# mishapadidar/GP-Derivatives-Variational-Inference

Measured on NVIDIA B200. Metric: DSVGP train points/s (ELBO fwd+bwd), higher is better.
Workload: dtype f32

## Files before the change

gp-derivatives-variational-inference_b200/csrc/api.cu:

```cuda
#include "../../include/dsvgp_b200.h"
#include "chol.cuh"
#include "common.cuh"
#include "data.cuh"
#include "gemm.cuh"
#include "kdir.cuh"
#include "misc.cuh"
#include "optim.cuh"
#include "tc_prep.cuh"
#include "trmm_tc.cuh"

using namespace dsvgp;
#define ST(s) reinterpret_cast<cudaStream_t>(s)

namespace dsvgp { unsigned long long g_launch_count = 0; }
namespace dsvgp { extern int g_fwd_tib, g_fwd_stream_stores, g_bwd_vpl; }

extern "C" {

int dsvgp_version(void) { return 100; }
int64_t dsvgp_launch_count(void) { return (int64_t)dsvgp::g_launch_count; }
int dsvgp_set_kdir_bwd_vpl(int vpl) {
  if (vpl == 2 || vpl == 4) dsvgp::g_bwd_vpl = vpl;
  return dsvgp::g_bwd_vpl;
}
int dsvgp_set_kdir_fwd_knobs(int tib, int stream_stores) {
  const int old = dsvgp::g_fwd_tib * 4 + dsvgp::g_fwd_stream_stores;
  if (tib == 0 || (tib >= 8 && tib <= 64 && tib % 8 == 0)) dsvgp::g_fwd_tib = tib;
  if (stream_stores >= 0 && stream_stores <= 2) dsvgp::g_fwd_stream_stores = stream_stores;
  return old;
}
int dsvgp_built_for_sm(void) { return 100; }

int dsvgp_hyp_from_raw_f32(const float* a, const float* b, const float* c, const float* d, double* hyp, dsvgp_stream_t s) { return hyp_from_raw<float>(a, b, c, d, hyp, ST(s)); }
int dsvgp_hyp_from_raw_f64(const double* a, const double* b, const double* c, const double* d, double* hyp, dsvgp_stream_t s) { return hyp_from_raw<double>(a, b, c, d, hyp, ST(s)); }

int dsvgp_normalize_dirs_f32(const float* v, int rows, int d, float* vh, float* inv, dsvgp_stream_t s) { return normalize_dirs<float, float>(v, rows, d, vh, inv, ST(s)); }
int dsvgp_normalize_dirs_f64(const double* v, int rows, int d, double* vh, double* inv, dsvgp_stream_t s) { return normalize_dirs<double, double>(v, rows, d, vh, inv, ST(s)); }
int dsvgp_normalize_dirs_f32f64(const float* v, int rows, int d, double* vh, double* inv, dsvgp_stream_t s) { return normalize_dirs<float, double>(v, rows, d, vh, inv, ST(s)); }

int dsvgp_normalize_dirs_canon_f32(const float* v, int rows, int d, float* vh, float* inv, int* cidx, int* canon_flag, dsvgp_stream_t s) {
  if (!cidx || !canon_flag) return DSVGP_ERR_ARG;
  return normalize_dirs<float, float>(v, rows, d, vh, inv, ST(s), cidx, canon_flag);
}
int dsvgp_kdir_fwd_canon_f32(const float* x1, const float* u1, int n1, int p1, const float* x2, const float* w2, const int* cidx2, const int* canon_flag, int n2, int p2, int d, const double* hyp, int use_os, double diag_add, float* K, int64_t ldk, float* Klo, dsvgp_stream_t s) {
  if (!x1 || !x2 || !hyp || !K || (p1 > 0 && !u1) || (p2 > 0 && !w2)) return DSVGP_ERR_ARG;
  return kdir_fwd<float, float>(x1, u1, n1, p1, x2, w2, n2, p2, d, hyp, use_os, diag_add, K, ldk, ST(s), cidx2, canon_flag, Klo);
}

#define KFWD(NAME, T, TK)                                                                                          \
  int NAME(const T* x1, const TK* u1, int n1, int p1, const T* x2, const TK* w2, int n2, int p2, int d,            \
           const double* hyp, int use_os, double diag_add, TK* K, int64_t ldk, dsvgp_stream_t s) {                 \
    if (!x1 || !x2 || !hyp || !K || (p1 > 0 && !u1) || (p2 > 0 && !w2)) return DSVGP_ERR_ARG;                     \
    return kdir_fwd<T, TK>(x1, u1, n1, p1, x2, w2, n2, p2, d, hyp, use_os, diag_add, K, ldk, ST(s));               \
  }
KFWD(dsvgp_kdir_fwd_f32, float, float)
KFWD(dsvgp_kdir_fwd_f64, double, double)
KFWD(dsvgp_kdir_fwd_f32f64, float, double)

int dsvgp_kdir_diag_f32(int n, int p, const double* hyp, int use_os, float* out, dsvgp_stream_t s) { return kdir_diag<float>(n, p, hyp, use_os, out, ST(s)); }
int dsvgp_kdir_diag_f64(int n, int p, const double* hyp, int use_os, double* out, dsvgp_stream_t s) { return kdir_diag<double>(n, p, hyp, use_os, out, ST(s)); }

size_t dsvgp_kdir_bwd_workspace_f32(int n1, int p1, int n2, int p2, int d) { return kdir_bwd_workspace<float>(n1, p1, n2, p2, d); }
size_t dsvgp_kdir_bwd_workspace_f64(int n1, int p1, int n2, int p2, int d) { return kdir_bwd_workspace<double>(n1, p1, n2, p2, d); }

#define KBWD(NAME, T, TK)                                                                                          \
  int NAME(const T* x1, const TK* u1, const TK* inv1, int n1, int p1, const T* x2, const TK* w2, int n2, int p2,   \
           int d, const double* hyp, int use_os, const TK* dK, int64_t lddk, int dk_trans, double scale,           \
           double* gx, double* gv, double* gsc, void* ws, size_t ws_bytes, dsvgp_stream_t s) {                     \
                                                \
    if (!x1 || !x2 || !hyp || !dK || !ws || (p1 > 0 && (!u1 || (gv && !inv1))) || (p2 > 0 && !w2)) return DSVGP_ERR_ARG; \
    return kdir_bwd<T, TK>(x1, u1, inv1, n1, p1, x2, w2, n2, p2, d, hyp, use_os, dK, lddk, dk_trans, scale, gx,    \
                           gv, gsc, ws, ws_bytes, ST(s));                                                          \
  }
KBWD(dsvgp_kdir_bwd_f32, float, float)
KBWD(dsvgp_kdir_bwd_f64, double, double)
KBWD(dsvgp_kdir_bwd_f32f64, float, double)

void dsvgp_chol_plan(int Mq, int* Mp, int* nb0, int* nlev) { chol_plan(Mq, Mp, nb0, nlev); }
int dsvgp_pad_identity_f64(double* A, int64_t ld, int Mq, int Mp, dsvgp_stream_t s) { return pad_identity(A, ld, Mq, Mp, ST(s)); }
int dsvgp_chol_f64(double* Awork, int64_t lda, double* L, int64_t ldl, double* W, int64_t ldw, int Mp, int nb0, int nlev, int* info, dsvgp_stream_t s) {
  return chol_factor_inverse(Awork, lda, L, ldl, W, ldw, Mp, nb0, nlev, info, ST(s));
}

int dsvgp_set_potrf_debug(void* p) { set_potrf_debug(static_cast<long long*>(p)); return 0; }
int dsvgp_collect_grads_f32(const double* small, int nZ, int nV, const double* hyp, int noise_mode, float* out, dsvgp_stream_t s) { return collect_grads<float>(small, nZ, nV, hyp, noise_mode, out, ST(s)); }
int dsvgp_collect_grads_f64(const double* small, int nZ, int nV, const double* hyp, int noise_mode, double* out, dsvgp_stream_t s) { return collect_grads<double>(small, nZ, nV, hyp, noise_mode, out, ST(s)); }
int dsvgp_set_gemm64_async(int on) { set_gemm64_async(on); return get_gemm64_async(); }
int dsvgp_set_rank_update(int on) { set_rank_update(on); return get_rank_update(); }
int dsvgp_set_chol_variant(int v) { set_chol_variant(v); return get_chol_variant(); }
int dsvgp_set_chol_lookahead(int on) { set_chol_lookahead(on); return get_chol_lookahead(); }
int dsvgp_set_chol_mid_link(int k) { set_chol_mid_link(k); return get_chol_mid_link(); }
int dsvgp_chol_wait_mid(dsvgp_stream_t s) { return chol_wait_mid(reinterpret_cast<cudaStream_t>(s)); }
int dsvgp_set_chol_inv_streams(int n) { set_chol_inv_streams(n); return get_chol_inv_streams(); }
int dsvgp_set_chol_graph(int on) { set_chol_graph(on); return get_chol_graph(); }
int dsvgp_set_chol_priority(int on) { set_chol_priority(on); return get_chol_priority(); }

int dsvgp_gemm_f32(int ta, int tb, int M, int N, int K, double alpha, const float* A, int64_t lda, const float* B, int64_t ldb, double beta, float* C, int64_t ldc, int a_tri, int b_tri, int c_tri, int batch, int64_t sA, int64_t sB, int64_t sC, const float* D, int64_t ldd, float* C2, int64_t ldc2, const float* D2, int64_t ldd2, dsvgp_stream_t s) {
  return gemm<float>(ta != 0, tb != 0, M, N, K, (float)alpha, A, lda, B, ldb, (float)beta, C, ldc, a_tri, b_tri, c_tri, batch, sA, sB, sC, ST(s), D, ldd, C2, ldc2, D2, ldd2);
}
int dsvgp_gemm_f64(int ta, int tb, int M, int N, int K, double alpha, const double* A, int64_t lda, const double* B, int64_t ldb, double beta, double* C, int64_t ldc, int a_tri, int b_tri, int c_tri, int batch, int64_t sA, int64_t sB, int64_t sC, const double* D, int64_t ldd, double* C2, int64_t ldc2, const double* D2, int64_t ldd2, dsvgp_stream_t s) {
  return gemm<double>(ta != 0, tb != 0, M, N, K, alpha, A, lda, B, ldb, beta, C, ldc, a_tri, b_tri, c_tri, batch, sA, sB, sC, ST(s), D, ldd, C2, ldc2, D2, ldd2);
}

int dsvgp_absmax_f32(const float* x, int64_t ld, int rows, int cols, int mode, unsigned int* out_bits, dsvgp_stream_t s) { return absmax<float>(x, ld, rows, cols, mode, out_bits, ST(s)); }
int dsvgp_absmax_f64(const double* x, int64_t ld, int rows, int cols, int mode, unsigned int* out_bits, dsvgp_stream_t s) { return absmax<double>(x, ld, rows, cols, mode, out_bits, ST(s)); }
int dsvgp_tc_scales_f32(const double* hyp, double jitter, const unsigned int* maxbits, int Mq, float* scales, int stage, dsvgp_stream_t s) { return tc_scales(hyp, jitter, maxbits, Mq, scales, stage, ST(s)); }
int dsvgp_split_half_f32(const float* src, int64_t lds, int rows, int cols, int mode, const float* scale, void* hi, void* lo, int64_t ldh, void* hiT, void* loT, int64_t ldhT, dsvgp_stream_t s) { return split_half<float>(src, lds, rows, cols, mode, scale, hi, lo, ldh, hiT, loT, ldhT, ST(s)); }
int dsvgp_split_half_f64(const double* src, int64_t lds, int rows, int cols, int mode, const float* scale, void* hi, void* lo, int64_t ldh, void* hiT, void* loT, int64_t ldhT, dsvgp_stream_t s) { return split_half<double>(src, lds, rows, cols, mode, scale, hi, lo, ldh, hiT, loT, ldhT, ST(s)); }
int dsvgp_build_d_split_f32(const float* E, int64_t lde, const float* P, int64_t ldp, int n, const float* scale, void* hi, void* lo, int64_t ldh, dsvgp_stream_t s) { return build_d_split(E, lde, P, ldp, n, scale, hi, lo, ldh, ST(s)); }
int dsvgp_build_d_absmax_f32(const float* E, int64_t lde, const float* P, int64_t ldp, int n, unsigned int* out_bits, dsvgp_stream_t s) { return build_d_absmax(E, lde, P, ldp, n, out_bits, ST(s)); }
int dsvgp_kdir_fwd_half_f32(const float* x1, const float* u1, int n1, int p1, const float* x2, const float* w2, const int* cidx2, const int* canon_flag, int n2, int p2, int d, const double* hyp, int use_os, double diag_add, float* K, int64_t ldk, void* Kh, void* Kl, int64_t ldkh, const float* hscale, dsvgp_stream_t s) {
  if (!x1 || !x2 || !hyp || !K || !Kh || !Kl || !hscale || (p1 > 0 && !u1) || (p2 > 0 && !w2)) return DSVGP_ERR_ARG;
  return kdir_fwd<float, float>(x1, u1, n1, p1, x2, w2, n2, p2, d, hyp, use_os, diag_add, K, ldk, ST(s), cidx2, canon_flag, nullptr, Kh, Kl, ldkh, hscale);
}
int dsvgp_dA_half_f32(const float* A, const float* C, int64_t ld, int rows, int nq, const float* m, const float* gmu, const float* gvar, float* tp, int nslab, float* t, void* dAh, void* dAl, void* Agh, void* Agl, int64_t ldh, const float* s_dA, const float* s_Ag, dsvgp_stream_t s) {
  if (!A || !C || !m || !gmu || !gvar || !tp || !t || !dAh || !dAl || !Agh || !Agl || !s_dA || !s_Ag) return DSVGP_ERR_ARG;
  return dA_apply_half(A, C, ld, rows, nq, m, gmu, gvar, tp, nslab, t, dAh, dAl, Agh, Agl, ldh, s_dA, s_Ag, nullptr, nullptr, nullptr, ST(s));
}
int dsvgp_dA_half_h_f32(const void* Ah, const void* Al, const float* a_scale, const float* C, int64_t ld, int rows, int nq, const float* m, const float* gmu, const float* gvar, float* tp, int nslab, float* t, void* dAh, void* dAl, void* Agh, void* Agl, int64_t ldh, const float* s_dA, const float* s_Ag, dsvgp_stream_t s) {
  if (!Ah || !Al || !a_scale || !C || !m || !gmu || !gvar || !tp || !t || !dAh || !dAl || !Agh || !Agl || !s_dA || !s_Ag) return DSVGP_ERR_ARG;
  return dA_apply_half(nullptr, C, ld, rows, nq, m, gmu, gvar, tp, nslab, t, dAh, dAl, Agh, Agl, ldh, s_dA, s_Ag, Ah, Al, a_scale, ST(s));
}
int dsvgp_col_dots_h_f32(const void* Ah, const void* Al, int64_t ldh, const float* a_scale, const float* C, int64_t ld, int rows, int nq, const float* m, float* pm, float* pv, int nslab, unsigned int* cmax_bits, dsvgp_stream_t s) {
  if (!m || !pm || !pv) return DSVGP_ERR_ARG;
  return col_dots_half(Ah, Al, ldh, a_scale, C, ld, rows, nq, m, pm, pv, nslab, cmax_bits, ST(s));
}
int dsvgp_gemm_tch_supported_f32(const void* A, int64_t lda, const void* B, int64_t ldb, int b_kmajor, int N) { return gemm_tch_supported(A, lda, B, ldb, b_kmajor, N); }
int dsvgp_gemm_tch_f32(const void* Ah, const void* Al, int64_t lda, const void* Bh, const void* Bl, int64_t ldb, int b_kmajor, int M, int N, int K, double alpha, double beta, const float* ab_inv, float* C, int64_t ldc, const float* D, int64_t ldd, float* C2, int64_t ldc2, const float* D2, int64_t ldd2, void* Ch, void* Cl, int64_t ldch, const float* c_scale, void* C2h, void* C2l, int64_t ldc2h, const float* c2_scale, int a_tri, int c_lower, int chunk, int nsplit, float* split_ws, dsvgp_stream_t s) {
  return gemm_tch(Ah, Al, lda, Bh, Bl, ldb, b_kmajor, M, N, K, (float)alpha, (float)beta, ab_inv, C, ldc, D, ldd, C2, ldc2, D2, ldd2, Ch, Cl, ldch, c_scale, C2h, C2l, ldc2h, c2_scale, a_tri, c_lower, chunk, nsplit, split_ws, ST(s));
}
int dsvgp_gemm_tc_supported_f32(const float* A, int64_t lda, const float* B, int64_t ldb, int b_kmajor, int N) { return gemm_tc_supported(A, lda, B, ldb, b_kmajor, N); }
int dsvgp_gemm_tc_f32(const float* Ah, const float* Al, int64_t lda, const float* Bh, const float* Bl, int64_t ldb, int b_kmajor, int M, int N, int K, double alpha, double beta, float* C, int64_t ldc, const float* D, int64_t ldd, float* C2, int64_t ldc2, const float* D2, int64_t ldd2, int a_tri, int c_lower, int chunk, float* Clo, float* C2lo, int nsplit, float* split_ws, dsvgp_stream_t s) {
  return gemm_tc(Ah, Al, lda, Bh, Bl, ldb, b_kmajor, M, N, K, (float)alpha, (float)beta, C, ldc, D, ldd, C2, ldc2, D2, ldd2, a_tri, c_lower, chunk, Clo, C2lo, nsplit, split_ws, ST(s));
}
int dsvgp_set_tc_tile_n(int n) { set_tc_tile_n(n); return get_tc_tile_n(); }
int dsvgp_set_tc_max_pairs(int n) { set_tc_max_pairs(n); return get_tc_max_pairs(); }
int dsvgp_set_tc_persistent(int on) { set_tc_persistent(on); return get_tc_persistent(); }
int dsvgp_set_tc_trace(void* buf, int cap_items) { set_tc_trace(static_cast<long long*>(buf), cap_items); return DSVGP_OK; }
int dsvgp_tc_work_list(int M, int N, int K, int a_tri, int c_lower, int nsplit, int pairs, int bke, int* out, int cap) {
  if (M <= 0 || N <= 0 || K <= 0 || nsplit < 1 || pairs < 1 || bke < 1 || cap < 0 || (cap > 0 && !out)) return DSVGP_ERR_ARG;
  const std::vector<int> t = tc::build_sched(M, N, K, a_tri, c_lower, nsplit, pairs, bke, nullptr);
  for (int i = 0; i < cap && i < (int)t.size(); ++i) out[i] = t[i];
  return (int)t.size();
}
int dsvgp_set_tc_cta_group(int cg) { set_tc_cta_group(cg); return get_tc_cta_group(); }
int dsvgp_split_lo_f32(const float* x, int64_t ldx, float* lo, int64_t ldl, int rows, int cols, dsvgp_stream_t s) { return split_lo(x, ldx, lo, ldl, rows, cols, ST(s)); }
int dsvgp_transpose_f32(const float* src, int64_t lds, float* dst, int64_t ldd, int rows, int cols, dsvgp_stream_t s) { return transpose_f32(src, lds, dst, ldd, rows, cols, ST(s)); }

// ... 73 lines not shown
```

gp-derivatives-variational-inference_b200/csrc/build.py:

```python
import os
import subprocess
import sys
from concurrent.futures import ThreadPoolExecutor

HERE = os.path.dirname(os.path.abspath(__file__))
OUT = os.path.join(os.path.dirname(HERE), "dsvgp_b200", "libdsvgp_b200.so")
SOURCES = ["kdir.cu", "gemm.cu", "chol.cu", "misc.cu", "optim.cu", "data.cu", "tc_prep.cu", "trmm_tc.cu", "api.cu"]
NVCC = os.environ.get("NVCC", "/usr/local/cuda/bin/nvcc")
FLAGS = ["-gencode", "arch=compute_100a,code=sm_100a", "-lineinfo", "-O3", "-std=c++17",
         "-Xcompiler", "-fPIC", "--expt-relaxed-constexpr"]


def _newer(a, b):
    return not os.path.exists(b) or os.path.getmtime(a) > os.path.getmtime(b)


def build(force=False, verbose=False):
    bdir = os.path.join(HERE, "build")
    os.makedirs(bdir, exist_ok=True)
    headers = [os.path.join(HERE, f) for f in os.listdir(HERE) if f.endswith((".cuh", ".h"))]
    headers.append(os.path.join(os.path.dirname(os.path.dirname(HERE)), "include", "dsvgp_b200.h"))
    srcs = [s for s in SOURCES if os.path.exists(os.path.join(HERE, s))]
    objs, jobs = [], []
    for s in srcs:
        src, obj = os.path.join(HERE, s), os.path.join(bdir, s[:-3] + ".o")
        objs.append(obj)
        if force or _newer(src, obj) or any(_newer(h, obj) for h in headers):
            jobs.append([NVCC, *FLAGS, *(["-Xptxas", "-v"] if verbose else []), "-c", src, "-o", obj])

    def run(cmd):
        r = subprocess.run(cmd, capture_output=True, text=True)
        if r.returncode != 0:
            raise RuntimeError("nvcc failed: " + " ".join(cmd) + "\n" + r.stdout + r.stderr)
        if verbose:
            sys.stderr.write(r.stderr)

    with ThreadPoolExecutor(max_workers=min(6, max(1, len(jobs)))) as ex:
        list(ex.map(run, jobs))
    if jobs or not os.path.exists(OUT):
        run([NVCC, "-shared", "-gencode", "arch=compute_100a,code=sm_100a", "-o", OUT, *objs])
    return OUT


if __name__ == "__main__":
    print(build(force="--force" in sys.argv, verbose="-v" in sys.argv))
```

gp-derivatives-variational-inference_b200/dsvgp_b200/_lib.py:

```python
import ctypes
import os
import re

import torch

_HERE = os.path.dirname(os.path.abspath(__file__))
LIB_PATH = os.path.join(_HERE, "libdsvgp_b200.so")
HEADER_PATH = os.path.normpath(os.path.join(_HERE, "..", "..", "include", "dsvgp_b200.h"))

_CTYPES = {"int": ctypes.c_int, "int64_t": ctypes.c_int64, "double": ctypes.c_double, "size_t": ctypes.c_size_t,
           "dsvgp_stream_t": ctypes.c_void_p, "void": None}
_PROTO = re.compile(r"^(int|void|size_t|int64_t)\s+(dsvgp_\w+)\s*\(([^;]*)\)\s*;", re.M)

ERRORS = {-1: "DSVGP_ERR_ARG (bad argument)", -2: "DSVGP_ERR_LAUNCH (CUDA launch failed)",
          -3: "DSVGP_ERR_WORKSPACE (workspace too small)"}


class DsvgpError(RuntimeError):
    pass


def parse_header(path=HEADER_PATH):
    protos = {}
    with open(path) as f:
        text = f.read()
    for ret, name, args in _PROTO.findall(text):
        argtypes = []
        args = args.strip()
        if args and args != "void":
            for a in args.split(","):
                a = a.strip()
                if "*" in a:
                    argtypes.append(ctypes.c_void_p)
                else:
                    argtypes.append(_CTYPES[a.replace("const ", "").split()[0]])
        protos[name] = (_CTYPES[ret], argtypes)
    return protos


PROTOTYPES = parse_header()

if not os.path.exists(LIB_PATH):
    raise ImportError(
        f"{LIB_PATH} is missing: build it with `python gp-derivatives-variational-inference_b200/csrc/build.py` "
        "(or __graft_entry__.build()).  dsvgp_b200 has no CPU or PyTorch fallback.")
_lib = ctypes.CDLL(LIB_PATH)
for _name, (_ret, _args) in PROTOTYPES.items():
    _fn = getattr(_lib, _name)
    _fn.restype = _ret
    _fn.argtypes = _args


def _arg(a):
    if a is None:
        return None
    if isinstance(a, torch.Tensor):
        if not a.is_cuda:
            raise DsvgpError("dsvgp_b200 kernels take CUDA tensors only (there is no CPU path)")
        return ctypes.c_void_p(a.data_ptr())
    return a


_RAW_STREAM = getattr(torch._C, "_cuda_getCurrentRawStream", None)
_GET_DEVICE = getattr(torch._C, "_cuda_getDevice", None)

# ... 56 lines not shown
```

gp-derivatives-variational-inference_b200/dsvgp_b200/engine.py:

```python
import os

import torch

from . import ops
from .ops import F32, F64, TRI_LOWER, TRI_UPPER

KZZ_JITTER = 1e-3
PRED_JITTER = 1e-4
CHOL_RETRY = (1e-6, 1e-5, 1e-4)
USE_TC = True
USE_FP16 = True
DENSE_D = True
WHITEN_FP64 = "auto"
WHITEN_FP64_MAX_NQ = 2048
DEFER_SIDE_WORK = True
TC_CHUNK = 2
TCH_CHUNK = 1
WORKSPACE_CACHE = 6
PERSISTENT_UNDER_REDUCE = os.environ.get("DSVGP_PERSISTENT_UNDER_REDUCE", "1") != "0"
HALF_A = False
F16 = torch.float16
_PARAM_NAMES = ("Z", "Vz", "m", "Ls_raw", "c", "raw_os", "raw_ell", "raw_noise")


# ... 70 lines not shown
        if self.tc:
            if not self.tch:
                self.lo1, self.lo2, self.lo3 = (e(Mq, self.ldn) for _ in range(3))
            self.E_lo, self.ET, self.ET_lo = sq(), sq(), sq()
            sg = lambda: e(Mq, self.ldg)[:, :Mq]
            self.G_lo, self.H_lo = sg(), sg()
            self.syrk_split = max(1, min(8, self.nq // 4096))
            self.split_ws = e(self.syrk_split * Mq * _round_up(Mq, 4)) if self.syrk_split > 1 else None
        self.nslab = max(1, ops.reduce_slabs(Mq, nq))
        self.pm, self.pv = e(self.nslab, nq), e(self.nslab, nq)
        self.mu, self.var, self.gmu, self.gvar = e(nq), e(nq), e(nq), e(nq)
        self.tp = e(max(1, min(64, nq // 2048)), Mq)
        self.big = torch.zeros(Mq * self.ldg + Mq, dtype=T, device=device)
        self.G, self.t = self.big[: Mq * self.ldg].view(Mq, self.ldg)[:, :Mq], self.big[Mq * self.ldg:]
        self.small = torch.zeros(8 + M * d + M * p * d, dtype=F64, device=device)
        self.sc = self.small[:8]
        self.gZ = self.small[8: 8 + M * d].view(M, d)
        self.gVz = self.small[8 + M * d:].view(M * p, d) if p else None
        self.small2 = torch.zeros_like(self.small)
        self.gZ2 = self.small2[8: 8 + M * d].view(M, d)
        self.gVz2 = self.small2[8 + M * d:].view(M * p, d) if p else None
        self.kl = torch.zeros(1, dtype=F64, device=device)
        self.scratch = e(max(8192, 2 * ((nq + 255) // 256) + 64), dt=F64)
        self.scratch_kl = e(512, dt=F64)
        self.H = e(Mq, self.ldg)[:, :Mq] if T == F32 else sq()
        self.X = sq()
        self.Y, self.Psi, self.S = (e(Mq, Mq, dt=F64) for _ in range(3))
        self.gm = self.gLs = None
        self.wx = None
        self.generation = 0
        self.canon = None


class Engine:
    def __init__(self):
        self._ws, self._fac, self._streams, self._events = {}, {}, {}, {}

    def _fork_event(self, device):
        key = str(device)
        ev = self._events.get(key)
        if ev is None:
            ev = self._events[key] = torch.cuda.Event()
        return ev

    def _scales_event(self, device):
        key = "scales:" + str(device)
        ev = self._events.get(key)
        if ev is None:
            ev = self._events[key] = torch.cuda.Event()
        return ev

    def _side_stream(self, device):
        key = str(device)
        st = self._streams.get(key)
        if st is None:
            st = self._streams[key] = torch.cuda.Stream(device=device)
        return st

    def workspace(self, device, dtype, n, d, M, p, p2):
        key = (str(device), dtype, n, d, M, p, p2)
        ws = self._ws.pop(key, None)
        if ws is None:
            while len(self._ws) >= WORKSPACE_CACHE:
                self._ws.pop(next(iter(self._ws)))
            ws = Workspace(device, dtype, n, d, M, p, p2)
        self._ws[key] = ws
        ws.generation += 1
        return ws

    def factor(self, device, dtype, d, M, p):
        key = (str(device), dtype, d, M, p)
        f = self._fac.pop(key, None)
        if f is None:
            while len(self._fac) >= WORKSPACE_CACHE:
                self._fac.pop(next(iter(self._fac)))
            f = Factor(device, dtype, d, M, p)
        self._fac[key] = f
        f.generation += 1
        return f

    @staticmethod
    def _validate(P, x, Vx, p, p2, y=None):
        if x.dim() != 2:
            raise ValueError(f"x must be (n, d); got {tuple(x.shape)}")
        if not x.is_cuda:
            raise TypeError("dsvgp_b200 runs on CUDA tensors only (there is no CPU path)")
        T, dev = x.dtype, x.device
        if T not in (F32, F64):
            raise TypeError(f"unsupported dtype {T}: the hot path is built for float32 and float64")
        n, d = x.shape
        M = P.Z.shape[0]
        Mq = M * (p + 1)
        want = {"Z": (M, d), "Vz": (M * p, d) if p else None, "m": (Mq,), "Ls_raw": (Mq, Mq)}
        for name in _PARAM_NAMES:
            t = getattr(P, name, None)
            if t is None:
                continue
            if t.dtype != T or t.device != dev:
                raise TypeError(f"parameter `{name}` is {t.dtype} on {t.device}, the inputs are {T} on {dev}: move the "
                                "model and the likelihood to the dtype / device of the data (model.to(...))")
            shp = want.get(name)
            if shp is not None and tuple(t.shape) != shp:
                raise ValueError(f"parameter `{name}` has shape {tuple(t.shape)}, expected {shp}")
            if name in ("Z", "Vz", "m", "Ls_raw") and not t.is_contiguous():
                raise ValueError(f"parameter `{name}` must be contiguous")
        if p2:
# ... 553 lines not shown
```

gp-derivatives-variational-inference_b200/dsvgp_b200/ops.py:

```python
import torch

from . import _lib
from ._lib import call, call_raw, suffix

TRI_NONE, TRI_LOWER, TRI_UPPER = 0, 1, 2
F32, F64 = torch.float32, torch.float64


def _ld(t):
    assert t.dim() == 2 and t.stride(1) == 1, "matrix operands must be row-major with unit inner stride"
    return t.stride(0)


def _pair_suffix(t_in, t_k):
    if t_in == t_k:
        return suffix(t_in)
    if t_in == F32 and t_k == F64:
        return "f32f64"
    raise _lib.DsvgpError(f"unsupported dtype pair {t_in}/{t_k}")


def hyp_from_raw(raw_ell, raw_os=None, raw_noise=None, c=None, out=None):
    out = torch.empty(8, dtype=F64, device=raw_ell.device) if out is None else out
    call("dsvgp_hyp_from_raw_" + suffix(raw_ell.dtype), raw_ell, raw_os, raw_noise, c, out)
# ... 70 lines not shown
    if N is None:
        N = B.shape[0] if tb else B.shape[1]
    call("dsvgp_gemm_" + suffix(C.dtype), int(ta), int(tb), M, N, K, float(alpha), A, _ld(A), B, _ld(B), float(beta),
         C, _ld(C), a_tri, b_tri, c_tri, 1, 0, 0, 0, D, _ld(D) if D is not None else 0,
         C2, _ld(C2) if C2 is not None else 0, D2, _ld(D2) if D2 is not None else 0)
    return C


def split_lo(x, lo=None, rows=None, cols=None):
    lo = torch.empty_like(x) if lo is None else lo
    call("dsvgp_split_lo_f32", x, _ld(x), lo, _ld(lo), x.shape[0] if rows is None else rows,
         x.shape[1] if cols is None else cols)
    return lo


def transpose(src, dst, rows=None, cols=None):
    call("dsvgp_transpose_f32", src, _ld(src), dst, _ld(dst), src.shape[0] if rows is None else rows,
         src.shape[1] if cols is None else cols)
    return dst


def set_rank_update(on):
    return call_raw("dsvgp_set_rank_update", int(on))


def set_chol_variant(v):
    return call_raw("dsvgp_set_chol_variant", int(v))


def set_chol_lookahead(on):
    return call_raw("dsvgp_set_chol_lookahead", int(bool(on)))


def set_chol_mid_link(k):
    return call_raw("dsvgp_set_chol_mid_link", int(k))


def chol_wait_mid():
    return call("dsvgp_chol_wait_mid")


def set_chol_inv_streams(n):
    return call_raw("dsvgp_set_chol_inv_streams", int(n))


def set_chol_graph(on):
    return call_raw("dsvgp_set_chol_graph", int(bool(on)))


def set_chol_priority(on):
    return call_raw("dsvgp_set_chol_priority", int(bool(on)))


def set_kdir_bwd_vpl(vpl):
    return call_raw("dsvgp_set_kdir_bwd_vpl", int(vpl))


def set_tc_cta_group(cg):
    return call_raw("dsvgp_set_tc_cta_group", int(cg))


def set_tc_tile_n(n):
    return call_raw("dsvgp_set_tc_tile_n", int(n))


def set_tc_max_pairs(n):
    return call_raw("dsvgp_set_tc_max_pairs", int(n))


def set_tc_persistent(on):
    return call_raw("dsvgp_set_tc_persistent", int(bool(on)))


def gemm_tch(A, B, C, M, N, K, ab_inv, b_kmajor=False, alpha=1.0, beta=0.0, D=None, C2=None, D2=None, Ch=None, c_scale=None,
             C2h=None, c2_scale=None, a_tri=TRI_NONE, c_lower=False, chunk=1, nsplit=1, split_ws=None):
    ld = lambda t: _ld(t) if t is not None else 0
    call("dsvgp_gemm_tch_f32", A[0], A[1], _ld(A[0]), B[0], B[1], _ld(B[0]), int(b_kmajor), M, N, K, float(alpha), float(beta),
         ab_inv, C, ld(C), D, ld(D), C2, ld(C2), D2, ld(D2), Ch[0] if Ch else None, Ch[1] if Ch else None,
         _ld(Ch[0]) if Ch else 0, c_scale, C2h[0] if C2h else None, C2h[1] if C2h else None, _ld(C2h[0]) if C2h else 0, c2_scale,
         a_tri, int(c_lower), chunk, int(nsplit), split_ws)
    return C


def absmax(x, out_bits, mode=0):
    x2 = x if x.dim() == 2 else x.reshape(1, -1)
    call("dsvgp_absmax_" + suffix(x.dtype), x2, _ld(x2), x2.shape[0], x2.shape[1], mode, out_bits)


def tc_scales(hyp, jitter, maxbits, Mq, scales, stage):
    call("dsvgp_tc_scales_f32", hyp, float(jitter), maxbits, int(Mq), scales, int(stage))


def split_half(src, scale, hi, lo, mode=0, hiT=None, loT=None, rows=None, cols=None):
    call("dsvgp_split_half_" + suffix(src.dtype), src, _ld(src), src.shape[0] if rows is None else rows,
         src.shape[1] if cols is None else cols, mode, scale, hi, lo, _ld(hi), hiT, loT, _ld(hiT) if hiT is not None else 0)


def build_d_split(E, P, scale, hi, lo, n=None):
    call("dsvgp_build_d_split_f32", E, _ld(E), P, _ld(P), E.shape[0] if n is None else n, scale, hi, lo, _ld(hi))


def build_d_absmax(E, P, out_bits, n=None):
    call("dsvgp_build_d_absmax_f32", E, _ld(E), P, _ld(P), E.shape[0] if n is None else n, out_bits)


def kdir_fwd_half(x1, u1, p1, x2, w2, p2, hyp, K, Kh, Kl, hscale, canon=None, use_os=True):
# ... 136 lines not shown
```

include/dsvgp_b200.h:

```cpp
#ifndef DSVGP_B200_H
#define DSVGP_B200_H

#include <stddef.h>
#include <stdint.h>

#ifdef __cplusplus
extern "C" {
#endif

typedef void* dsvgp_stream_t;

#define DSVGP_OK 0
#define DSVGP_ERR_ARG -1
#define DSVGP_ERR_LAUNCH -2
#define DSVGP_ERR_WORKSPACE -3

#define DSVGP_TRI_NONE 0
#define DSVGP_TRI_LOWER 1
#define DSVGP_TRI_UPPER 2

int dsvgp_version(void);
int dsvgp_built_for_sm(void);
int64_t dsvgp_launch_count(void);
int dsvgp_set_kdir_fwd_knobs(int tib, int stream_stores);
int dsvgp_set_kdir_bwd_vpl(int vpl);

int dsvgp_hyp_from_raw_f32(const float* raw_ell, const float* raw_os, const float* raw_noise, const float* c, double* hyp, dsvgp_stream_t s);
int dsvgp_hyp_from_raw_f64(const double* raw_ell, const double* raw_os, const double* raw_noise, const double* c, double* hyp, dsvgp_stream_t s);

int dsvgp_normalize_dirs_f32(const float* v, int rows, int d, float* vhat, float* inv_norm, dsvgp_stream_t s);
int dsvgp_normalize_dirs_f64(const double* v, int rows, int d, double* vhat, double* inv_norm, dsvgp_stream_t s);
int dsvgp_normalize_dirs_f32f64(const float* v, int rows, int d, double* vhat, double* inv_norm, dsvgp_stream_t s);

int dsvgp_kdir_fwd_f32(const float* x1, const float* u1, int n1, int p1, const float* x2, const float* w2, int n2, int p2, int d, const double* hyp, int use_os, double diag_add, float* K, int64_t ldk, dsvgp_stream_t s);
int dsvgp_kdir_fwd_f64(const double* x1, const double* u1, int n1, int p1, const double* x2, const double* w2, int n2, int p2, int d, const double* hyp, int use_os, double diag_add, double* K, int64_t ldk, dsvgp_stream_t s);
int dsvgp_kdir_fwd_f32f64(const float* x1, const double* u1, int n1, int p1, const float* x2, const double* w2, int n2, int p2, int d, const double* hyp, int use_os, double diag_add, double* K, int64_t ldk, dsvgp_stream_t s);

int dsvgp_normalize_dirs_canon_f32(const float* v, int rows, int d, float* vhat, float* inv_norm, int* cidx, int* canon_flag, dsvgp_stream_t s);
int dsvgp_kdir_fwd_canon_f32(const float* x1, const float* u1, int n1, int p1, const float* x2, const float* w2, const int* cidx2, const int* canon_flag, int n2, int p2, int d, const double* hyp, int use_os, double diag_add, float* K, int64_t ldk, float* Klo, dsvgp_stream_t s);

int dsvgp_kdir_diag_f32(int n, int p, const double* hyp, int use_os, float* out, dsvgp_stream_t s);
int dsvgp_kdir_diag_f64(int n, int p, const double* hyp, int use_os, double* out, dsvgp_stream_t s);

size_t dsvgp_kdir_bwd_workspace_f32(int n1, int p1, int n2, int p2, int d);
size_t dsvgp_kdir_bwd_workspace_f64(int n1, int p1, int n2, int p2, int d);
int dsvgp_kdir_bwd_f32(const float* x1, const float* u1, const float* inv1, int n1, int p1, const float* x2, const float* w2, int n2, int p2, int d, const double* hyp, int use_os, const float* dK, int64_t lddk, int dk_trans, double scale, double* gx, double* gv, double* gsc, void* ws, size_t ws_bytes, dsvgp_stream_t s);
int dsvgp_kdir_bwd_f64(const double* x1, const double* u1, const double* inv1, int n1, int p1, const double* x2, const double* w2, int n2, int p2, int d, const double* hyp, int use_os, const double* dK, int64_t lddk, int dk_trans, double scale, double* gx, double* gv, double* gsc, void* ws, size_t ws_bytes, dsvgp_stream_t s);
int dsvgp_kdir_bwd_f32f64(const float* x1, const double* u1, const double* inv1, int n1, int p1, const float* x2, const double* w2, int n2, int p2, int d, const double* hyp, int use_os, const double* dK, int64_t lddk, int dk_trans, double scale, double* gx, double* gv, double* gsc, void* ws, size_t ws_bytes, dsvgp_stream_t s);

void dsvgp_chol_plan(int Mq, int* Mp_host, int* nb0_host, int* nlev_host);
int dsvgp_pad_identity_f64(double* A, int64_t ld, int Mq, int Mp, dsvgp_stream_t s);
int dsvgp_set_chol_variant(int v);
int dsvgp_set_chol_priority(int on);
int dsvgp_set_chol_mid_link(int k);
int dsvgp_chol_wait_mid(dsvgp_stream_t s);
int dsvgp_set_chol_graph(int on);
int dsvgp_set_chol_inv_streams(int n);
int dsvgp_set_chol_lookahead(int on);
int dsvgp_set_potrf_debug(void* buf);
int dsvgp_chol_f64(double* Awork, int64_t lda, double* L, int64_t ldl, double* W, int64_t ldw, int Mp, int nb0, int nlev, int* info, dsvgp_stream_t s);

int dsvgp_gemm_f32(int ta, int tb, int M, int N, int K, double alpha, const float* A, int64_t lda, const float* B, int64_t ldb, double beta, float* C, int64_t ldc, int a_tri, int b_tri, int c_tri, int batch, int64_t sA, int64_t sB, int64_t sC, const float* D, int64_t ldd, float* C2, int64_t ldc2, const float* D2, int64_t ldd2, dsvgp_stream_t s);
int dsvgp_gemm_f64(int ta, int tb, int M, int N, int K, double alpha, const double* A, int64_t lda, const double* B, int64_t ldb, double beta, double* C, int64_t ldc, int a_tri, int b_tri, int c_tri, int batch, int64_t sA, int64_t sB, int64_t sC, const double* D, int64_t ldd, double* C2, int64_t ldc2, const double* D2, int64_t ldd2, dsvgp_stream_t s);

int dsvgp_set_gemm64_async(int on);
int dsvgp_set_rank_update(int on);

int dsvgp_gemm_tc_supported_f32(const float* A, int64_t lda, const float* B, int64_t ldb, int b_kmajor, int N);
int dsvgp_gemm_tc_f32(const float* Ah, const float* Al, int64_t lda, const float* Bh, const float* Bl, int64_t ldb, int b_kmajor, int M, int N, int K, double alpha, double beta, float* C, int64_t ldc, const float* D, int64_t ldd, float* C2, int64_t ldc2, const float* D2, int64_t ldd2, int a_tri, int c_lower, int chunk, float* Clo, float* C2lo, int nsplit, float* split_ws, dsvgp_stream_t s);
int dsvgp_gemm_tch_supported_f32(const void* A, int64_t lda, const void* B, int64_t ldb, int b_kmajor, int N);
int dsvgp_gemm_tch_f32(const void* Ah, const void* Al, int64_t lda, const void* Bh, const void* Bl, int64_t ldb, int b_kmajor, int M, int N, int K, double alpha, double beta, const float* ab_inv, float* C, int64_t ldc, const float* D, int64_t ldd, float* C2, int64_t ldc2, const float* D2, int64_t ldd2, void* Ch, void* Cl, int64_t ldch, const float* c_scale, void* C2h, void* C2l, int64_t ldc2h, const float* c2_scale, int a_tri, int c_lower, int chunk, int nsplit, float* split_ws, dsvgp_stream_t s);
int dsvgp_absmax_f32(const float* x, int64_t ld, int rows, int cols, int mode, unsigned int* out_bits, dsvgp_stream_t s);
int dsvgp_absmax_f64(const double* x, int64_t ld, int rows, int cols, int mode, unsigned int* out_bits, dsvgp_stream_t s);
int dsvgp_tc_scales_f32(const double* hyp, double jitter, const unsigned int* maxbits, int Mq, float* scales, int stage, dsvgp_stream_t s);
int dsvgp_split_half_f32(const float* src, int64_t lds, int rows, int cols, int mode, const float* scale, void* hi, void* lo, int64_t ldh, void* hiT, void* loT, int64_t ldhT, dsvgp_stream_t s);
int dsvgp_split_half_f64(const double* src, int64_t lds, int rows, int cols, int mode, const float* scale, void* hi, void* lo, int64_t ldh, void* hiT, void* loT, int64_t ldhT, dsvgp_stream_t s);
int dsvgp_build_d_split_f32(const float* E, int64_t lde, const float* P, int64_t ldp, int n, const float* scale, void* hi, void* lo, int64_t ldh, dsvgp_stream_t s);
int dsvgp_build_d_absmax_f32(const float* E, int64_t lde, const float* P, int64_t ldp, int n, unsigned int* out_bits, dsvgp_stream_t s);
int dsvgp_kdir_fwd_half_f32(const float* x1, const float* u1, int n1, int p1, const float* x2, const float* w2, const int* cidx2, const int* canon_flag, int n2, int p2, int d, const double* hyp, int use_os, double diag_add, float* K, int64_t ldk, void* Kh, void* Kl, int64_t ldkh, const float* hscale, dsvgp_stream_t s);
int dsvgp_dA_half_f32(const float* A, const float* C, int64_t ld, int rows, int nq, const float* m, const float* gmu, const float* gvar, float* tp, int nslab, float* t, void* dAh, void* dAl, void* Agh, void* Agl, int64_t ldh, const float* s_dA, const float* s_Ag, dsvgp_stream_t s);
int dsvgp_dA_half_h_f32(const void* Ah, const void* Al, const float* a_scale, const float* C, int64_t ld, int rows, int nq, const float* m, const float* gmu, const float* gvar, float* tp, int nslab, float* t, void* dAh, void* dAl, void* Agh, void* Agl, int64_t ldh, const float* s_dA, const float* s_Ag, dsvgp_stream_t s);
int dsvgp_col_dots_h_f32(const void* Ah, const void* Al, int64_t ldh, const float* a_scale, const float* C, int64_t ld, int rows, int nq, const float* m, float* pm, float* pv, int nslab, unsigned int* cmax_bits, dsvgp_stream_t s);
int dsvgp_set_tc_cta_group(int cg);
int dsvgp_set_tc_tile_n(int n);
int dsvgp_set_tc_persistent(int on);
int dsvgp_set_tc_max_pairs(int n);
int dsvgp_set_tc_trace(void* buf, int cap_items);
int dsvgp_tc_work_list(int M, int N, int K, int a_tri, int c_lower, int nsplit, int pairs, int bke, int* out, int cap);
int dsvgp_split_lo_f32(const float* x, int64_t ldx, float* lo, int64_t ldl, int rows, int cols, dsvgp_stream_t s);
int dsvgp_transpose_f32(const float* src, int64_t lds, float* dst, int64_t ldd, int rows, int cols, dsvgp_stream_t s);

int dsvgp_cast_f64_f32(const double* src, int64_t lds, float* dst, int64_t ldd, int rows, int cols, int tril, dsvgp_stream_t s);
int dsvgp_cast_f32_f64(const float* src, int64_t lds, double* dst, int64_t ldd, int rows, int cols, int tril, dsvgp_stream_t s);
int dsvgp_cast_f64_f64(const double* src, int64_t lds, double* dst, int64_t ldd, int rows, int cols, int tril, dsvgp_stream_t s);
int dsvgp_cast_f32_f32(const float* src, int64_t lds, float* dst, int64_t ldd, int rows, int cols, int tril, dsvgp_stream_t s);
int dsvgp_mirror_lower_f32(float* A, int64_t ld, int n, dsvgp_stream_t s);
int dsvgp_mirror_lower_f64(double* A, int64_t ld, int n, dsvgp_stream_t s);
int dsvgp_add_outer_f32(float* A, int64_t ld, int n, const float* u, const float* v, double alpha, dsvgp_stream_t s);
int dsvgp_add_outer_f64(double* A, int64_t ld, int n, const double* u, const double* v, double alpha, dsvgp_stream_t s);
int dsvgp_tril_minus_eye_f32(const float* Ls, int64_t ldl, float* E, int64_t lde, int n, dsvgp_stream_t s);
int dsvgp_tril_minus_eye_f64(const double* Ls, int64_t ldl, double* E, int64_t lde, int n, dsvgp_stream_t s);
int dsvgp_sym_phi_f64(const double* Y, int64_t ldy, double* P, int64_t ldp, int n, dsvgp_stream_t s);
int dsvgp_phi_lower_f64(const double* Y, int64_t ldy, double* P, int64_t ldp, int n, dsvgp_stream_t s);
int dsvgp_symmetrize_f64(double* A, int64_t ld, int n, dsvgp_stream_t s);
int dsvgp_phi_outer_f32(const float* X, int64_t ldx, const float* u, const float* v, double* P, int64_t ldp, int n, dsvgp_stream_t s);
int dsvgp_phi_outer_f64(const double* X, int64_t ldx, const double* u, const double* v, double* P, int64_t ldp, int n, dsvgp_stream_t s);
// ... 40 lines not shown
```

Baseline: 1.497 million.

## Run side-stream filler work on a green-context SM partition

```diff
diff --git a/gp-derivatives-variational-inference_b200/csrc/api.cu b/gp-derivatives-variational-inference_b200/csrc/api.cu
--- a/gp-derivatives-variational-inference_b200/csrc/api.cu
+++ b/gp-derivatives-variational-inference_b200/csrc/api.cu
@@ -6,6 +6,7 @@
 #include "kdir.cuh"
 #include "misc.cuh"
 #include "optim.cuh"
+#include "partition.cuh"
 #include "tc_prep.cuh"
 #include "trmm_tc.cuh"
 
@@ -94,6 +95,12 @@
 int dsvgp_set_chol_inv_streams(int n) { set_chol_inv_streams(n); return get_chol_inv_streams(); }
 int dsvgp_set_chol_graph(int on) { set_chol_graph(on); return get_chol_graph(); }
 int dsvgp_set_chol_priority(int on) { set_chol_priority(on); return get_chol_priority(); }
+dsvgp_stream_t dsvgp_filler_stream(void) { return filler_stream(); }
+int dsvgp_set_filler_sms(int n) {
+  if (n >= 0 && n % 8 != 0) return DSVGP_ERR_ARG;
+  set_filler_sms(n);
+  return get_filler_sms();
+}
 
 int dsvgp_gemm_f32(int ta, int tb, int M, int N, int K, double alpha, const float* A, int64_t lda, const float* B, int64_t ldb, double beta, float* C, int64_t ldc, int a_tri, int b_tri, int c_tri, int batch, int64_t sA, int64_t sB, int64_t sC, const float* D, int64_t ldd, float* C2, int64_t ldc2, const float* D2, int64_t ldd2, dsvgp_stream_t s) {
   return gemm<float>(ta != 0, tb != 0, M, N, K, (float)alpha, A, lda, B, ldb, (float)beta, C, ldc, a_tri, b_tri, c_tri, batch, sA, sB, sC, ST(s), D, ldd, C2, ldc2, D2, ldd2);
diff --git a/gp-derivatives-variational-inference_b200/csrc/build.py b/gp-derivatives-variational-inference_b200/csrc/build.py
--- a/gp-derivatives-variational-inference_b200/csrc/build.py
+++ b/gp-derivatives-variational-inference_b200/csrc/build.py
@@ -5,7 +5,7 @@
 
 HERE = os.path.dirname(os.path.abspath(__file__))
 OUT = os.path.join(os.path.dirname(HERE), "dsvgp_b200", "libdsvgp_b200.so")
-SOURCES = ["kdir.cu", "gemm.cu", "chol.cu", "misc.cu", "optim.cu", "data.cu", "tc_prep.cu", "trmm_tc.cu", "api.cu"]
+SOURCES = ["kdir.cu", "gemm.cu", "chol.cu", "misc.cu", "optim.cu", "data.cu", "tc_prep.cu", "trmm_tc.cu", "partition.cu", "api.cu"]
 NVCC = os.environ.get("NVCC", "/usr/local/cuda/bin/nvcc")
 FLAGS = ["-gencode", "arch=compute_100a,code=sm_100a", "-lineinfo", "-O3", "-std=c++17",
          "-Xcompiler", "-fPIC", "--expt-relaxed-constexpr"]
diff --git a/gp-derivatives-variational-inference_b200/csrc/partition.cu b/gp-derivatives-variational-inference_b200/csrc/partition.cu
--- /dev/null
+++ b/gp-derivatives-variational-inference_b200/csrc/partition.cu
@@ -0,0 +1,129 @@
+#include <cuda.h>
+
+#include "common.cuh"
+
+namespace dsvgp {
+namespace {
+
+typedef CUresult (*GetDevResourceFn)(CUdevice, CUdevResource*, CUdevResourceType);
+typedef CUresult (*SplitByCountFn)(CUdevResource*, unsigned int*, const CUdevResource*, CUdevResource*, unsigned int, unsigned int);
+typedef CUresult (*GenerateDescFn)(CUdevResourceDesc*, CUdevResource*, unsigned int);
+typedef CUresult (*GreenCtxCreateFn)(CUgreenCtx*, CUdevResourceDesc, CUdevice, unsigned int);
+typedef CUresult (*GreenCtxDestroyFn)(CUgreenCtx);
+typedef CUresult (*GreenCtxStreamCreateFn)(CUstream*, CUgreenCtx, unsigned int, int);
+typedef CUresult (*StreamSyncFn)(CUstream);
+typedef CUresult (*StreamDestroyFn)(CUstream);
+
+struct Driver {
+  GetDevResourceFn get_resource = nullptr;
+  SplitByCountFn split = nullptr;
+  GenerateDescFn gen_desc = nullptr;
+  GreenCtxCreateFn ctx_create = nullptr;
+  GreenCtxDestroyFn ctx_destroy = nullptr;
+  GreenCtxStreamCreateFn stream_create = nullptr;
+  StreamSyncFn stream_sync = nullptr;
+  StreamDestroyFn stream_destroy = nullptr;
+  bool ok = false;
+};
+
+template <typename F>
+bool entry(const char* name, F* fn) {
+  void* p = nullptr;
+  cudaDriverEntryPointQueryResult q;
+  if (cudaGetDriverEntryPoint(name, &p, cudaEnableDefault, &q) != cudaSuccess || q != cudaDriverEntryPointSuccess || !p) {
+    cudaGetLastError();
+    return false;
+  }
+  *fn = reinterpret_cast<F>(p);
+  return true;
+}
+
+const Driver& driver() {
+  static Driver d;
+  static bool tried = false;
+  if (!tried) {
+    tried = true;
+    d.ok = entry("cuDeviceGetDevResource", &d.get_resource) && entry("cuDevSmResourceSplitByCount", &d.split) &&
+           entry("cuDevResourceGenerateDesc", &d.gen_desc) && entry("cuGreenCtxCreate", &d.ctx_create) &&
+           entry("cuGreenCtxDestroy", &d.ctx_destroy) && entry("cuGreenCtxStreamCreate", &d.stream_create) &&
+           entry("cuStreamSynchronize", &d.stream_sync) && entry("cuStreamDestroy", &d.stream_destroy);
+  }
+  return d;
+}
+
+struct Partition {
+  bool tried = false;
+  CUgreenCtx ctx = nullptr;
+  CUstream stream = nullptr;
+};
+
+Partition g_parts[16];
+int g_filler_sms = 0;
+
+void release(Partition& p) {
+  const Driver& d = driver();
+  if (p.stream) {
+    d.stream_sync(p.stream);
+    d.stream_destroy(p.stream);
+  }
+  if (p.ctx) d.ctx_destroy(p.ctx);
+  p = Partition{};
+}
+
+struct ReleaseAtUnload {
+  ~ReleaseAtUnload() {
+    if (!driver().ok) return;
+    for (Partition& p : g_parts)
+      if (p.ctx) release(p);
+  }
+} g_release_at_unload;
+
+}
+
+int filler_sms_default(int sms) {
+  const int n = (sms - 36) & ~7;
+  return n >= 8 ? n : 0;
+}
+
+void set_filler_sms(int n) {
+  if (n == g_filler_sms) return;
+  g_filler_sms = n;
+  if (!driver().ok) return;
+  for (Partition& p : g_parts)
+    if (p.tried) release(p);
+}
+
+int get_filler_sms() { return g_filler_sms; }
+
+cudaStream_t filler_stream() {
+  int dev = 0;
+  if (cudaGetDevice(&dev) != cudaSuccess || dev >= 16) return nullptr;
+  Partition& p = g_parts[dev];
+  if (p.tried) return reinterpret_cast<cudaStream_t>(p.stream);
+  p.tried = true;
+  const Driver& d = driver();
+  if (!d.ok || g_filler_sms < 0) return nullptr;
+  int sms = 0;
+  cudaDeviceGetAttribute(&sms, cudaDevAttrMultiProcessorCount, dev);
+  const int want = g_filler_sms > 0 ? g_filler_sms : filler_sms_default(sms);
+  if (want < 8 || want % 8 != 0 || want >= sms) return nullptr;
+  CUdevResource all{}, part{}, rest{};
+  unsigned int groups = 1;
+  CUdevResourceDesc desc = nullptr;
+  if (d.get_resource((CUdevice)dev, &all, CU_DEV_RESOURCE_TYPE_SM) != CUDA_SUCCESS ||
+      d.split(&part, &groups, &all, &rest, 0, (unsigned)want) != CUDA_SUCCESS || groups != 1 ||
+      part.sm.smCount != (unsigned)want || d.gen_desc(&desc, &part, 1) != CUDA_SUCCESS ||
+      d.ctx_create(&p.ctx, desc, (CUdevice)dev, CU_GREEN_CTX_DEFAULT_STREAM) != CUDA_SUCCESS) {
+    p.ctx = nullptr;
+    return nullptr;
+  }
+  if (d.stream_create(&p.stream, p.ctx, CU_STREAM_NON_BLOCKING, 0) != CUDA_SUCCESS) {
+    d.ctx_destroy(p.ctx);
+    p.ctx = nullptr;
+    p.stream = nullptr;
+    return nullptr;
+  }
+  return reinterpret_cast<cudaStream_t>(p.stream);
+}
+
+}
diff --git a/gp-derivatives-variational-inference_b200/csrc/partition.cuh b/gp-derivatives-variational-inference_b200/csrc/partition.cuh
--- /dev/null
+++ b/gp-derivatives-variational-inference_b200/csrc/partition.cuh
@@ -0,0 +1,9 @@
+#pragma once
+#include <cuda_runtime.h>
+
+namespace dsvgp {
+int filler_sms_default(int sms);
+void set_filler_sms(int n);
+int get_filler_sms();
+cudaStream_t filler_stream();
+}
diff --git a/gp-derivatives-variational-inference_b200/dsvgp_b200/_lib.py b/gp-derivatives-variational-inference_b200/dsvgp_b200/_lib.py
--- a/gp-derivatives-variational-inference_b200/dsvgp_b200/_lib.py
+++ b/gp-derivatives-variational-inference_b200/dsvgp_b200/_lib.py
@@ -10,7 +10,7 @@
 
 _CTYPES = {"int": ctypes.c_int, "int64_t": ctypes.c_int64, "double": ctypes.c_double, "size_t": ctypes.c_size_t,
            "dsvgp_stream_t": ctypes.c_void_p, "void": None}
-_PROTO = re.compile(r"^(int|void|size_t|int64_t)\s+(dsvgp_\w+)\s*\(([^;]*)\)\s*;", re.M)
+_PROTO = re.compile(r"^(int|void|size_t|int64_t|dsvgp_stream_t)\s+(dsvgp_\w+)\s*\(([^;]*)\)\s*;", re.M)
 
 ERRORS = {-1: "DSVGP_ERR_ARG (bad argument)", -2: "DSVGP_ERR_LAUNCH (CUDA launch failed)",
           -3: "DSVGP_ERR_WORKSPACE (workspace too small)"}
diff --git a/gp-derivatives-variational-inference_b200/dsvgp_b200/engine.py b/gp-derivatives-variational-inference_b200/dsvgp_b200/engine.py
--- a/gp-derivatives-variational-inference_b200/dsvgp_b200/engine.py
+++ b/gp-derivatives-variational-inference_b200/dsvgp_b200/engine.py
@@ -146,6 +146,13 @@
 
     def _side_stream(self, device):
         key = str(device)
+        if not torch.cuda.is_current_stream_capturing():
+            h = ops.filler_stream()
+            if h:
+                st = self._streams.get("filler:" + key)
+                if st is None or st.cuda_stream != h:
+                    st = self._streams["filler:" + key] = torch.cuda.ExternalStream(h, device=device)
+                return st
         st = self._streams.get(key)
         if st is None:
             st = self._streams[key] = torch.cuda.Stream(device=device)
diff --git a/gp-derivatives-variational-inference_b200/dsvgp_b200/ops.py b/gp-derivatives-variational-inference_b200/dsvgp_b200/ops.py
--- a/gp-derivatives-variational-inference_b200/dsvgp_b200/ops.py
+++ b/gp-derivatives-variational-inference_b200/dsvgp_b200/ops.py
@@ -146,6 +146,14 @@
     return call_raw("dsvgp_set_chol_priority", int(bool(on)))
 
 
+def filler_stream():
+    return call_raw("dsvgp_filler_stream")
+
+
+def set_filler_sms(n):
+    return call_raw("dsvgp_set_filler_sms", int(n))
+
+
 def set_kdir_bwd_vpl(vpl):
     return call_raw("dsvgp_set_kdir_bwd_vpl", int(vpl))
 
diff --git a/include/dsvgp_b200.h b/include/dsvgp_b200.h
--- a/include/dsvgp_b200.h
+++ b/include/dsvgp_b200.h
@@ -52,6 +52,8 @@
 int dsvgp_pad_identity_f64(double* A, int64_t ld, int Mq, int Mp, dsvgp_stream_t s);
 int dsvgp_set_chol_variant(int v);
 int dsvgp_set_chol_priority(int on);
+dsvgp_stream_t dsvgp_filler_stream(void);
+int dsvgp_set_filler_sms(int n);
 int dsvgp_set_chol_mid_link(int k);
 int dsvgp_chol_wait_mid(dsvgp_stream_t s);
 int dsvgp_set_chol_graph(int on);
diff --git a/scratch/green_probe.py b/scratch/green_probe.py
--- /dev/null
+++ b/scratch/green_probe.py
@@ -0,0 +1,147 @@
+import ctypes, os, sys, time
+ROOT = os.path.dirname(os.path.dirname(os.path.abspath(__file__)))
+sys.path.insert(0, ROOT); sys.path.insert(0, os.path.join(ROOT, "gp-derivatives-variational-inference_b200"))
+import torch
+from dsvgp_b200 import ops, _lib
+from dsvgp_b200.ops import TRI_LOWER
+
+dev = torch.device("cuda", 0)
+torch.cuda.init(); torch.zeros(1, device=dev)
+print("device", torch.cuda.get_device_name(0), "SMs", torch.cuda.get_device_properties(0).multi_processor_count, flush=True)
+os.system("nvidia-smi --query-gpu=name,power.limit,clocks.max.sm --format=csv,noheader")
+
+h = ops.filler_stream()
+print("filler_stream", hex(h or 0), "filler_sms in force", ops.set_filler_sms(0), flush=True)
+assert h, "no filler partition"
+
+cu = ctypes.CDLL("libcuda.so.1")
+all_, part, rest = (ctypes.create_string_buffer(144) for _ in range(3))
+assert cu.cuDeviceGetDevResource(0, all_, 1) == 0
+ng = ctypes.c_uint(1)
+assert cu.cuDevSmResourceSplitByCount(part, ctypes.byref(ng), all_, rest, 0, 128) == 0
+sm = lambda b: int.from_bytes(b.raw[96:100], "little")
+print("split: all", sm(all_), "part", sm(part), "rest", sm(rest), flush=True)
+desc = ctypes.c_void_p(); gctx = ctypes.c_void_p(); rs = ctypes.c_void_p()
+assert cu.cuDevResourceGenerateDesc(ctypes.byref(desc), rest, 1) == 0
+assert cu.cuGreenCtxCreate(ctypes.byref(gctx), desc, 0, 1) == 0
+assert cu.cuGreenCtxStreamCreate(ctypes.byref(rs), gctx, 1, 0) == 0
+S_part = torch.cuda.ExternalStream(h, device=dev)
+S_rest = torch.cuda.ExternalStream(rs.value, device=dev)
+S_prim = torch.cuda.Stream(device=dev)
+
+
+def check(name, ok):
+    print(("OK   " if ok else "FAIL ") + name, flush=True)
+
+
+g = torch.Generator(device="cpu").manual_seed(0)
+x = torch.randn(4096, 4096, generator=g).to(dev)
+ref = (x * 3 + 1).sin()
+for nm, S in (("partition", S_part), ("remainder", S_rest)):
+    with torch.cuda.stream(S):
+        y = (x * 3 + 1).sin()
+    S.synchronize()
+    check(f"torch elementwise on {nm}", torch.equal(y, ref))
+
+Mq, nq = 3072, 8192
+A = torch.randn(Mq, Mq, generator=g).tril().to(dev)
+B = torch.randn(Mq, nq, generator=g).to(dev)
+A_lo, B_lo = ops.split_lo(A), ops.split_lo(B)
+
+
+def prod(S, persistent, pairs=0):
+    C = torch.full((Mq, nq), float("nan"), device=dev)
+    ops.set_tc_persistent(persistent); ops.set_tc_max_pairs(pairs)
+    with torch.cuda.stream(S):
+        ops.gemm_tc(A, A_lo, B, B_lo, C, Mq, nq, Mq, a_tri=TRI_LOWER, chunk=2)
+    S.synchronize()
+    ops.set_tc_persistent(True); ops.set_tc_max_pairs(0)
+    return C
+
+
+C0 = prod(S_prim, False)
+for nm, S, pairs in (("partition", S_part, 64), ("remainder", S_rest, 10)):
+    check(f"2-CTA gemm_tc per tile on {nm}", torch.equal(prod(S, False), C0))
+    check(f"2-CTA gemm_tc persistent ({pairs} pairs) on {nm}", torch.equal(prod(S, True, pairs), C0))
+
+
+def timeit(S, fn, reps=5):
+    with torch.cuda.stream(S):
+        fn()
+        e0, e1 = torch.cuda.Event(enable_timing=True), torch.cuda.Event(enable_timing=True)
+        e0.record(S)
+        for _ in range(reps): fn()
+        e1.record(S)
+    S.synchronize()
+    return e0.elapsed_time(e1) / reps
+
+
+Cx = torch.empty(Mq, nq, device=dev)
+ops.set_tc_persistent(False)
+f = lambda: ops.gemm_tc(A, A_lo, B, B_lo, Cx, Mq, nq, Mq, a_tri=TRI_LOWER, chunk=2)
+print("per-tile product ms: primary %.3f partition %.3f remainder %.3f" % (timeit(S_prim, f), timeit(S_part, f), timeit(S_rest, f)), flush=True)
+ops.set_tc_persistent(True)
+
+Mp, nb0, nlev = ops.chol_plan(Mq)
+Z = torch.randn(Mp, Mp + 64, generator=g, dtype=torch.float64).to(dev)
+K = (Z @ Z.T) / Mp + torch.eye(Mp, dtype=torch.float64, device=dev)
+
+
+def chol(S):
+    Aw, L, W = K.clone(), torch.zeros_like(K), torch.zeros_like(K)
+    info = torch.zeros(1, dtype=torch.int32, device=dev)
+    torch.cuda.synchronize()
+    with torch.cuda.stream(S):
+        ops.cholesky_inverse(Aw, L, W, nb0, nlev, info)
+    S.synchronize(); torch.cuda.synchronize()
+    return L, W, int(info)
+
+
+L0, W0, i0 = chol(S_prim)
+for nm, S in (("partition", S_part), ("remainder", S_rest)):
+    L1, W1, i1 = chol(S)
+    check(f"4-CTA potrf_cluster chain on {nm} (info {i1})", i1 == 0 and torch.equal(L1, L0) and torch.equal(W1, W0))
+
+for a_nm, Sa, b_nm, Sb in (("primary", S_prim, "partition", S_part), ("partition", S_part, "primary", S_prim)):
+    buf = torch.zeros(1 << 20, device=dev); out = torch.empty_like(buf)
+    ev = torch.cuda.Event()
+    torch.cuda.synchronize()
+    with torch.cuda.stream(Sa):
+        torch.cuda._sleep(100_000_000)
+        buf.fill_(7.0)
+        ev.record(Sa)
+    Sb.wait_event(ev)
+    with torch.cuda.stream(Sb):
+        out.copy_(buf)
+    Sb.synchronize()
+    check(f"event {a_nm} -> {b_nm}", bool((out == 7.0).all()))
+
+Aw, L, W = K.clone(), torch.zeros_like(K), torch.zeros_like(K)
+info = torch.zeros(1, dtype=torch.int32, device=dev)
+done = torch.zeros(1, device=dev)
+torch.cuda.synchronize()
+ops.cholesky_inverse(Aw, L, W, nb0, nlev, info)
+with torch.cuda.stream(S_part):
+    ops.chol_wait_mid()
+    done.fill_(1.0)
+torch.cuda.synchronize()
+check("chol_wait_mid on partition", float(done) == 1.0)
+
+try:
+    gx = torch.ones(1 << 20, device=dev); gy = torch.empty_like(gx)
+    cs = torch.cuda.Stream(device=dev)
+    graph = torch.cuda.CUDAGraph()
+    torch.cuda.synchronize()
+    with torch.cuda.graph(graph, stream=cs):
+        S_part.wait_stream(cs)
+        with torch.cuda.stream(S_part):
+            gy.copy_(gx * 5)
+        cs.wait_stream(S_part)
+    gx.fill_(2.0); graph.replay(); torch.cuda.synchronize()
+    check("graph capture forking into the partition", bool((gy == 10.0).all()))
+except Exception as e:
+    print("FAIL graph capture forking into the partition:", type(e).__name__, str(e)[:300], flush=True)
+    torch.cuda.synchronize()
+
+cu.cuStreamSynchronize(rs); cu.cuStreamDestroy_v2(rs); cu.cuGreenCtxDestroy(gctx)
+print("probe done", flush=True)
diff --git a/scratch/sm_partition_ab.py b/scratch/sm_partition_ab.py
--- /dev/null
+++ b/scratch/sm_partition_ab.py
@@ -0,0 +1,135 @@
+import os, statistics, sys
+ROOT = os.path.dirname(os.path.dirname(os.path.abspath(__file__)))
+sys.path.insert(0, ROOT); sys.path.insert(0, os.path.join(ROOT, "gp-derivatives-variational-inference_b200"))
+import torch, bench
+from dsvgp_b200 import gp, ops, engine
+
+dev = torch.device("cuda", 0)
+os.system("nvidia-smi --query-gpu=name,power.limit,clocks.max.sm --format=csv,noheader")
+
+_ev = {}
+_chol, _wait, _kl = ops.cholesky_inverse, ops.chol_wait_mid, ops.kl_divergence
+
+
+def _mark(name):
+    e = torch.cuda.Event(enable_timing=True); e.record(); _ev[name] = e
+
+
+def chol_hook(*a, **k):
+    _mark("chol0"); r = _chol(*a, **k); _mark("chol1"); return r
+
+
+def wait_hook(*a, **k):
+    r = _wait(*a, **k); _mark("fill0"); return r
+
+
+def kl_hook(*a, **k):
+    r = _kl(*a, **k); _mark("fill1"); return r
+
+
+EET_PAIRS = 0
+_set_pers = ops.set_tc_persistent
+
+
+def set_pers_hook(on):
+    if EET_PAIRS:
+        ops.set_tc_max_pairs(0 if on else EET_PAIRS)
+        return _set_pers(True)
+    return _set_pers(on)
+
+
+ops.set_tc_persistent = set_pers_hook
+
+
+def problem(name, n):
+    wl = dict(bench.WORKLOADS[name]); dtype = torch.float64 if wl["dtype"] == "f64" else torch.float32
+    model, lik = bench.build_model(wl, dtype, dev)
+    mll = gp.VariationalELBO(lik, model, num_data=(wl["d"] + 1) * wl["N"])
+    x, V, y = (t.to(dev) for t in bench.synth_batch(n, wl["d"], wl["p"], wl["variant"], dtype, "cpu", 1000))
+    params = list(model.parameters()) + list(lik.parameters())
+
+    def step():
+        for q in params: q.grad = None
+        loss = -mll(lik(model(x, derivative_directions=V)), y); loss.backward(); return loss
+    return step
+
+
+def time_steps(step, reps=20):
+    for _ in range(3): step()
+    torch.cuda.synchronize()
+    e0, e1 = torch.cuda.Event(enable_timing=True), torch.cuda.Event(enable_timing=True)
+    e0.record()
+    for _ in range(reps): step()
+    e1.record(); torch.cuda.synchronize()
+    return e0.elapsed_time(e1) / reps
+
+
+def spans(step):
+    ops.cholesky_inverse, ops.chol_wait_mid, ops.kl_divergence = chol_hook, wait_hook, kl_hook
+    try:
+        _ev.clear(); step(); torch.cuda.synchronize()
+        t = lambda k: _ev["chol0"].elapsed_time(_ev[k]) if k in _ev else float("nan")
+        return "chain 0-%.3f filler %.3f-%.3f" % (t("chol1"), t("fill0"), t("fill1"))
+    except RuntimeError as e:
+        return "spans n/a (%s)" % str(e)[:80]
+    finally:
+        ops.cholesky_inverse, ops.chol_wait_mid, ops.kl_divergence = _chol, _wait, _kl
+
+
+def run(name, n, settings, rounds=3):
+    step = problem(name, n)
+    res = {s[0]: [] for s in settings}
+    sp = {}
+    global EET_PAIRS
+    for r in range(rounds):
+        for label, sms, mid, eet in settings:
+            ops.set_filler_sms(sms); ops.set_chol_mid_link(mid); EET_PAIRS = eet
+            res[label].append(time_steps(step))
+            if r == 0:
+                sp[label] = spans(step)
+    ops.set_filler_sms(0); ops.set_chol_mid_link(20); EET_PAIRS = 0
+    for label, *_ in settings:
+        v = res[label]
+        print(f"{name} n={n:6d} {label:>18s}: median {statistics.median(v):.3f} ms  [{min(v):.3f} .. {max(v):.3f}]  {sp[label]}", flush=True)
+    del step
+    torch.cuda.empty_cache()
+
+
+SIZES = [("off", -1, 20, 0)] + [(f"part {s}", s, 20, 0) for s in (112, 120, 128, 136)]
+quick = len(sys.argv) > 1 and sys.argv[1] == "quick"
+if quick:
+    run("C3", 16384, SIZES[:1] + [("part default", 0, 20, 0)], rounds=3)
+    sys.exit(0)
+if len(sys.argv) > 1 and sys.argv[1] == "knobs":
+    def knob(label, prio=0, la=0, ru=0, mid=20, sms=0):
+        return (label, sms, mid, 0, prio, la, ru)
+    KN = [knob("off", sms=-1), knob("part"), knob("part prio", prio=1), knob("part prio mid14", prio=1, mid=14),
+          knob("part lookahead", la=1), knob("part rank_update2", ru=2), knob("off prio", prio=1, sms=-1)]
+    for name, n in (("C3", 16384), ("C3", 512), ("C5", 16384)):
+        step = problem(name, n)
+        res = {k[0]: [] for k in KN}
+        for r in range(3):
+            for label, sms, mid, _, prio, la, ru in KN:
+                ops.set_filler_sms(sms); ops.set_chol_mid_link(mid); ops.set_chol_priority(prio)
+                ops.set_chol_lookahead(la); ops.set_rank_update(ru)
+                res[label].append(time_steps(step))
+        ops.set_filler_sms(0); ops.set_chol_mid_link(20); ops.set_chol_priority(0); ops.set_chol_lookahead(0); ops.set_rank_update(0)
+        for label in res:
+            v = res[label]
+            print(f"{name} n={n:6d} {label:>18s}: median {statistics.median(v):.3f} ms  [{min(v):.3f} .. {max(v):.3f}]", flush=True)
+        del step
+        torch.cuda.empty_cache()
+    sys.exit(0)
+if len(sys.argv) > 1 and sys.argv[1] == "small":
+    SMALL = [("off", -1, 20, 0)] + [(f"part {s} mid {m}", s, m, 0) for s in (64, 80, 96, 104, 112) for m in (14, 20)]
+    run("C3", 16384, SMALL)
+    run("C3", 512, SMALL)
+    run("C5", 16384, SMALL[:1] + [x for x in SMALL[1:] if x[2] == 20])
+    run("C4", 2048, SMALL[:1] + [x for x in SMALL[1:] if x[2] == 20])
+    sys.exit(0)
+run("C3", 16384, SIZES + [(f"part0 mid {m}", 0, m, 0) for m in (8, 12, 16, 24)] + [("part0 EET pers", 0, 20, 64)])
+run("C3", 512, SIZES + [(f"part0 mid {m}", 0, m, 0) for m in (8, 12, 16, 24)])
+run("C3", 4096, SIZES)
+run("C2", 4096, SIZES)
+run("C4", 2048, SIZES)
+run("C5", 16384, SIZES)
```

Result: faster. 1.520 million, median of 6 (+1.5%).
